# weikaolun/horovod-distributed-example

Hardware: AMD Instinct MI355X
Metric: images/sec (whole node) + scaling efficiency, ResNet-50 bf16 at 1/2/4/8 MI355X (higher is better)
Workload: dtype bf16; 1 GPU; model=ResNet-50, global_batch=2048, per_gpu_batch=2048, image=224, parallelism=dp1, optimizer=mivod FusedSGD via DistributedOptimizer, compression=none, transport=local, hip_graph=False

## Files before the change

### csrc/kernels/mv_gemm256.hip

```cpp
#include "mv_mfma.h"
#include "mv_gemm.h"

#include <cstdio>
#include <cstdlib>
#include <string>

namespace mv {
namespace g256 {

constexpr int BM = 256, BN = 256, BK = 64, NT = 512;
constexpr int HALF = 128 * BK;
constexpr int BUF = 4 * HALF;

#ifndef MV_G256_DIAG
#define MV_G256_DIAG 0
#endif
template <int N>
__device__ __forceinline__ void wait_vm() {
  if constexpr (!(MV_G256_DIAG & 1) || N == 0)
    mv::wait_vm<N>();
}
__device__ __forceinline__ void barrier() {
  if constexpr (MV_G256_DIAG & 8) return;
  __builtin_amdgcn_sched_barrier(0);
  raw_barrier();
  __builtin_amdgcn_sched_barrier(0);
}

struct Args {
  const __bf16* A;
  const __bf16* A2;
  const __bf16* B;
  __bf16* C;
  int64_t M;
  int N, K, K1, ntn;
  int64_t ntiles;
  int ds, H, W, Ho, Wo;
  int Cin, ks;
  int ph, pw, Kb;
  const float* shift;
  float* partial;
  const float* badd;
  const __bf16* xb;
  const float* mean;
  const float* sc;
  const float* bi;
  uint32_t abytes, a2bytes, bbytes;
  const __bf16* bias16;
};

struct Pixel {
  uint32_t n, ho, wo;
};
__device__ __forceinline__ Pixel pixel_of(uint32_t r, int Ho, int Wo) {
  const uint32_t hw = (uint32_t)(Ho * Wo);
  const uint32_t n = r / hw, rem = r - n * hw;
  const uint32_t ho = rem / (uint32_t)Wo;
  return Pixel{n, ho, rem - ho * (uint32_t)Wo};
}

template <int EPI>
constexpr int nvec() { return EPI == 1 ? 1 : EPI == 4 ? 4 : (EPI == 6 || EPI == 7) ? 1 : 0; }
constexpr int kVecFloats = 8192;

template <int EPI, int AMODE, int MT>
__global__ __launch_bounds__(NT, 1) void gemm256_kernel(Args p) {
  constexpr bool DM = AMODE == 3 || AMODE == 4;
  constexpr int BMv = MT * 32;
  constexpr int MH1 = MT - 4;
  constexpr int NV = nvec<EPI>();
  constexpr bool STATS = EPI == 1 || EPI == 4 || EPI == 7;
  constexpr bool BADD = EPI == 4 || EPI == 6;
  constexpr bool XB = EPI == 4 || EPI == 7;
  __shared__ __attribute__((aligned(16))) __bf16 smem[2 * BUF + (NV ? 2 * kVecFloats : 0)];
  float* vecs = reinterpret_cast<float*>(smem + 2 * BUF);
  float* stacc = vecs + 4 * BN;
  const int N = p.N;
  const int tid = threadIdx.x, lane = tid & 63;
  const int w = __builtin_amdgcn_readfirstlane(tid >> 6);
  const int wm = w >> 2, wn = w & 3;
  const int G = gridDim.x;
  int64_t tile = xcd_remap(blockIdx.x, G);
  if (tile >= p.ntiles) return;
  const int64_t tile0 = tile;
  const int nw0 = (int)(tile0 % p.ntn) * BN;

  uint32_t offa[2][2], offb[2][2];
  uint32_t offa2[2][2];
  uint32_t abase[2][2];
  uint32_t avalid[2];
  const uint32_t scb = (uint32_t)(((lane & 7) ^ ((lane >> 3) & 7)) * 16);
  const int KT = p.K / BK, KT1 = AMODE == 2 ? p.K1 / BK : KT;
  const int csteps = (AMODE == 3 || AMODE == 4) ? p.Cin / BK : 1;
  const bool cpow2 = (csteps & (csteps - 1)) == 0;
  const int cshift = __builtin_ctz((unsigned)csteps);
  auto set_src = [&](int64_t tl) {
    const int64_t mt = tl / p.ntn;
    const int nt = (int)(tl - mt * p.ntn);
#pragma unroll
    for (int i = 0; i < 2; ++i) {
      const int r = (2 * w + i) * 8 + (lane >> 3);
      const int sc = (lane & 7) ^ (r & 7);
#pragma unroll
      for (int h = 0; h < 2; ++h) {
        const int rr = (r & 63);
        int64_t row = mt * BMv + (r >> 6) * (MT * 16) + h * 64 +
                      ((h == 1 && rr >= 16 * MH1) ? rr - 16 * MH1 : rr);
        row = row < p.M ? row : p.M - 1;
        if constexpr (AMODE == 1) {
          const Pixel px = pixel_of((uint32_t)row, p.Ho, p.Wo);
          const int64_t n = px.n;
          const int ho = (int)px.ho, wo = (int)px.wo;
          row = (n * p.H + (int64_t)ho * p.ds) * p.W + (int64_t)wo * p.ds;
        }
        if constexpr (AMODE == 3) {
          const Pixel px = pixel_of((uint32_t)row, p.Ho, p.Wo);
          const int64_t n = px.n;
          const int ho = (int)px.ho, wo = (int)px.wo;
          const int pad = p.ks >> 1;
          const int hi0 = ho * p.ds - pad, wi0 = wo * p.ds - pad;
          uint32_t v = 0;
#pragma unroll
          for (int tr = 0; tr < 3; ++tr)
#pragma unroll
            for (int ts = 0; ts < 3; ++ts) {
              const bool ok = tr < p.ks && ts < p.ks && (unsigned)(hi0 + tr) < (unsigned)p.H &&
                              (unsigned)(wi0 + ts) < (unsigned)p.W;
              v |= (ok ? 1u : 0u) << (tr * p.ks + ts);
            }
          if (i == 0) avalid[h] = v;
          else avalid[h] |= v << 16;
          abase[h][i] =
              (uint32_t)(((((int64_t)n * p.H + hi0) * p.W + wi0) * p.Cin + sc * 8) * 2);
        }
        if constexpr (AMODE == 4) {
          const uint32_t hw = (uint32_t)(p.Ho * p.Wo);
          const int rem = (int)((uint32_t)row % hw);
          const int ci = (int)((uint32_t)rem / (uint32_t)p.Wo), cj = rem - ci * p.Wo;
          const bool r1 = ci + 1 < p.Ho, c1 = cj + 1 < p.Wo;
          const uint32_t v = 1u | (c1 ? 2u : 0u) | (r1 ? 4u : 0u) | (r1 && c1 ? 8u : 0u);
          if (i == 0) avalid[h] = v;
          else avalid[h] |= v << 16;
          abase[h][i] = (uint32_t)((row * p.Cin + sc * 8) * 2);
        }
        if constexpr (AMODE == 2) {
          offa[h][i] = (uint32_t)(row * (p.K1 * 2)) + scb;
          int64_t row2 = row;
          if (p.ds > 1) {
            const Pixel px = pixel_of((uint32_t)row, p.Ho, p.Wo);
            const int64_t n = px.n;
            const int ho = (int)px.ho, wo = (int)px.wo;
            row2 = (n * p.H + (int64_t)ho * p.ds) * p.W + (int64_t)wo * p.ds;
          }
          offa2[h][i] = (uint32_t)(row2 * ((p.K - p.K1) * 2)) + scb;
        } else {
          offa[h][i] = (uint32_t)((row * p.K + sc * 8) * 2);
        }
        const int col = nt * BN + (r >> 5) * 64 + h * 32 + (r & 31);
        offb[h][i] = (uint32_t)(((int64_t)col * (AMODE == 4 ? p.Kb : p.K) + sc * 8) * 2);
      }
    }
  };
  const __amdgpu_buffer_rsrc_t rsA = buffer_rsrc(p.A, p.abytes);
  const __amdgpu_buffer_rsrc_t rsA2 =
      buffer_rsrc(AMODE == 2 ? p.A2 : p.A, AMODE == 2 ? p.a2bytes : 0u);
  const __amdgpu_buffer_rsrc_t rsB = buffer_rsrc(p.B, p.bbytes);
  struct KInfo {
    uint32_t toff, boff;
    int tap;
  };
  auto kinfo = [&](int kt) -> KInfo {
    uint32_t toff = 0, boff = kt * (BK * 2);
    int tap = 0;
    if constexpr (AMODE == 3) {
      tap = cpow2 ? kt >> cshift : kt / csteps;
      const int c0 = (kt - tap * csteps) * BK;
      const int tr = p.ks == 3 ? (tap * 11) >> 5 : tap / p.ks;
      const int ts = tap - tr * p.ks;
      toff = (uint32_t)(((tr * p.W + ts) * p.Cin + c0) * 2);
    }
    if constexpr (AMODE == 4) {
      const int t = cpow2 ? kt >> cshift : kt / csteps;
      const int c0 = (kt - t * csteps) * BK;
      const int tR = p.pw ? t >> 1 : t, tS = p.pw ? t & 1 : 0;
      const int rr = p.ph ? 2 * tR : 1, ss = p.pw ? 2 * tS : 1;
      tap = 2 * tR + tS;
      toff = (uint32_t)(((tR * p.Wo + tS) * p.Cin + c0) * 2);
      boff = (uint32_t)(((rr * 3 + ss) * p.Cin + c0) * 2);
    }
    return KInfo{toff, boff, tap};
  };
  auto issue_k = [&](int slot, int buf, int kt, const KInfo& ki, int ione) {
    if ((MV_G256_DIAG & 2) && kt != 0) return;
    const uint32_t toff = ki.toff, boff = ki.boff;
    const int tap = ki.tap;
    const bool second = AMODE == 2 && kt >= KT1;
    auto one = [&](int i) {
      __bf16* dst = smem + buf * BUF + slot * HALF + (2 * w + i) * 512;
      uint32_t vo;
      if (slot >= 2) {
        vo = offb[slot - 2][i] + boff;
      } else if constexpr (AMODE == 3 || AMODE == 4) {
        vo = ((avalid[slot] >> (tap + 16 * i)) & 1u) ? abase[slot][i] + toff : 0xFFFFFFF0u;
      } else if constexpr (AMODE == 2) {
        vo = second ? offa2[slot][i] + (uint32_t)(kt - KT1) * (BK * 2)
                    : offa[slot][i] + (uint32_t)kt * (BK * 2);
      } else {
        vo = offa[slot][i] + (uint32_t)kt * (BK * 2);
      }
      blds16(slot >= 2 ? rsB : (second ? rsA2 : rsA), vo, dst);
    };
    if (ione >= 0) {
      one(ione);
    } else {
      one(0);
      one(1);
    }
  };
  auto issue = [&](int slot, int buf, int kt) { issue_k(slot, buf, kt, kinfo(kt), -1); };

  f32x4v acc[4][8];
#pragma unroll
  for (int a = 0; a < 4; ++a)
#pragma unroll
    for (int b = 0; b < 8; ++b) acc[a][b] = f32x4v{0.f, 0.f, 0.f, 0.f};
  bf16x8 af[4][2], bfr[2][2][2];
  const int rl = lane & 15, g = lane >> 4;

  int kt = 0;
  auto read_a = [&](int buf, int h) {
    if ((MV_G256_DIAG & 4) && kt != 0) return;
    const __bf16* base = smem + buf * BUF + h * HALF;
#pragma unroll
    for (int b = 0; b < 4; ++b)
      if (h == 0 || b < MH1)
#pragma unroll
        for (int kk = 0; kk < 2; ++kk)
          af[b][kk] =
              *reinterpret_cast<const bf16x8*>(base + swz64(wm * 64 + b * 16 + rl, kk * 4 + g));
  };
  auto read_b = [&](int buf, int h) {
    if ((MV_G256_DIAG & 4) && kt != 0) return;
    const __bf16* base = smem + buf * BUF + (2 + h) * HALF;
#pragma unroll
    for (int a = 0; a < 2; ++a)
#pragma unroll
      for (int kk = 0; kk < 2; ++kk)
        bfr[h][a][kk] =
            *reinterpret_cast<const bf16x8*>(base + swz64(wn * 32 + a * 16 + rl, kk * 4 + g));
  };
  auto mma = [&](int qm, int qn) {
    __builtin_amdgcn_s_setprio(1);
#pragma unroll
    for (int kk = 0; kk < 2; ++kk)
#pragma unroll
      for (int a = 0; a < 2; ++a)
#pragma unroll
        for (int b = 0; b < 4; ++b)
          if (qm == 0 || b < MH1)
            acc[qn * 2 + a][qm * 4 + b] = mfma(bfr[qn][a][kk], af[b][kk], acc[qn * 2 + a][qm * 4 + b]);
    __builtin_amdgcn_s_setprio(0);
  };
  auto mma_dm = [&](int qm0, int qn0, int qm1, int qn1, int npc, int step, auto&& piece) {
    __builtin_amdgcn_s_setprio(1);
    int t = 0;
#pragma unroll
    for (int h = 0; h < 2; ++h) {
      const int qm = h ? qm1 : qm0, qn = h ? qn1 : qn0;
#pragma unroll
      for (int kk = 0; kk < 2; ++kk)
#pragma unroll
        for (int a = 0; a < 2; ++a)
#pragma unroll
          for (int b = 0; b < 4; ++b)
            if (qm == 0 || b < MH1) {
              acc[qn * 2 + a][qm * 4 + b] =
                  mfma(bfr[qn][a][kk], af[b][kk], acc[qn * 2 + a][qm * 4 + b]);
              if (t >= 1 && (t - 1) % step == 0 && (t - 1) / step < npc) {
                __builtin_amdgcn_sched_barrier(0);
                piece((t - 1) / step);
                __builtin_amdgcn_sched_barrier(0);
              }
              ++t;
            }
    }
    __builtin_amdgcn_s_setprio(0);
  };
  auto out_row = [&](int64_t row) -> int64_t {
    if constexpr (AMODE != 4) {
      return row;
    } else {
      const Pixel px = pixel_of((uint32_t)row, p.Ho, p.Wo);
      return ((int64_t)px.n * p.H + 2 * px.ho + p.ph) * p.W + 2 * px.wo + p.pw;
    }
  };
  auto epilogue = [&](int64_t tl) {
    const int64_t mt = tl / p.ntn;
    const int n0 = (int)(tl - mt * p.ntn) * BN;
    const int64_t m0 = mt * BMv;
    float s1[2][8], s2[2][8];
#pragma unroll
    for (int q = 0; q < 2; ++q)
#pragma unroll
      for (int j = 0; j < 8; ++j) {
        s1[q][j] = 0.f;
        s2[q][j] = 0.f;
      }
    constexpr int XBB = EPI == 7 ? 4 : 2;
    uint4 xr[XBB][2];
#pragma unroll
    for (int b = 0; b < MT; ++b) {
      if (XB && (b % XBB) == 0) {
#pragma unroll
        for (int bb = 0; bb < XBB; ++bb) {
          const int64_t row = m0 + wm * (MT * 16) + (b + bb) * 16 + rl;
          const int64_t orow = out_row(row);
#pragma unroll
          for (int q = 0; q < 2; ++q) {
            const int c0 = n0 + wn * 64 + q * 32 + (g & 1) * 16 + (g >> 1) * 8;
            xr[bb][q] = (b + bb < MT && row < p.M) ? *reinterpret_cast<const uint4*>(p.xb + orow * N + c0)
                                  : uint4{0u, 0u, 0u, 0u};
          }
        }
      }
      const int64_t row = m0 + wm * (MT * 16) + b * 16 + rl;
      const bool in = row < p.M;
      const int64_t orow = out_row(row);
#pragma unroll
      for (int q = 0; q < 2; ++q) {
        f32x4v u = acc[2 * q][b], v = acc[2 * q + 1][b];
        if constexpr (BADD) {
          const int cu = n0 + wn * 64 + 2 * q * 16 + 4 * g;
          const f32x4v bu = *reinterpret_cast<const f32x4v*>(vecs + (cu - n0));
          const f32x4v bv = *reinterpret_cast<const f32x4v*>(vecs + (cu - n0) + 16);
          u += bu;
          v += bv;
        }
        uint32_t x0 = cvt_pk_bf16(u[0], u[1]), x1 = cvt_pk_bf16(u[2], u[3]);
        uint32_t y0 = cvt_pk_bf16(v[0], v[1]), y1 = cvt_pk_bf16(v[2], v[3]);
        const auto r0 = __builtin_amdgcn_permlane16_swap(x0, y0, false, false);
        const auto r1 = __builtin_amdgcn_permlane16_swap(x1, y1, false, false);
        uint32_t o[4] = {r0[0], r1[0], r0[1], r1[1]};
        const int c0 = n0 + wn * 64 + q * 32 + (g & 1) * 16 + (g >> 1) * 8;
        if constexpr (EPI == 1) {
          if (in) {
#pragma unroll
            for (int j = 0; j < 8; ++j) {
              const float f = (j & 1) ? __uint_as_float(o[j >> 1] & 0xffff0000u)
                                      : __uint_as_float(o[j >> 1] << 16);
              const float d = f - vecs[c0 - n0 + j];
              s1[q][j] += d;
              s2[q][j] += d * d;
            }
          }
        }
        if constexpr (EPI == 4) {
          if (in) {
            const uint32_t xw[4] = {xr[b % XBB][q].x, xr[b % XBB][q].y, xr[b % XBB][q].z, xr[b % XBB][q].w};
            const float* mean = vecs + BN - n0;
            const float* scv = vecs + 2 * BN - n0;
            const float* biv = vecs + 3 * BN - n0;
            float dv[8];
#pragma unroll
            for (int j = 0; j < 8; ++j) {
              const float f = (j & 1) ? __uint_as_float(o[j >> 1] & 0xffff0000u)
                                      : __uint_as_float(o[j >> 1] << 16);
              const float xv = (j & 1) ? __uint_as_float(xw[j >> 1] & 0xffff0000u)
                                       : __uint_as_float(xw[j >> 1] << 16);
              const float d = __builtin_fmaf(xv, scv[c0 + j], biv[c0 + j]) > 0.f ? f : 0.f;
              dv[j] = d;
              s1[q][j] += d;
              s2[q][j] += d * (xv - mean[c0 + j]);
            }
#pragma unroll
            for (int j = 0; j < 4; ++j) o[j] = cvt_pk_bf16(dv[2 * j], dv[2 * j + 1]);
          }
        }
        if constexpr (EPI == 7) {
          if (in) {
            const uint32_t xw[4] = {xr[b % XBB][q].x, xr[b % XBB][q].y, xr[b % XBB][q].z, xr[b % XBB][q].w};
            float dv[8];
#pragma unroll
            for (int j = 0; j < 8; ++j) {
              const float f = (j & 1) ? __uint_as_float(o[j >> 1] & 0xffff0000u)
                                      : __uint_as_float(o[j >> 1] << 16);
              const float xv = (j & 1) ? __uint_as_float(xw[j >> 1] & 0xffff0000u)
                                       : __uint_as_float(xw[j >> 1] << 16);
              const float d = f * gelu_grad(xv + vecs[c0 - n0 + j]);
              dv[j] = d;
              s1[q][j] += d;
            }
#pragma unroll
            for (int j = 0; j < 4; ++j) o[j] = cvt_pk_bf16(dv[2 * j], dv[2 * j + 1]);
          }
        }
        if (in && (EPI != 1 || p.C) && !(MV_G256_DIAG & 16)) {
          u32x4* dst = reinterpret_cast<u32x4*>(p.C + orow * N + c0);
          const u32x4 val{o[0], o[1], o[2], o[3]};
          if constexpr ((MV_G256_DIAG & 192) == 64) {
            __builtin_nontemporal_store(val, dst);
          } else if constexpr ((MV_G256_DIAG & 192) == 128) {
            asm volatile("global_store_dwordx4 %0, %1, off sc1" ::"v"(dst), "v"(val) : "memory");
          } else if constexpr ((MV_G256_DIAG & 192) == 192) {
            asm volatile("global_store_dwordx4 %0, %1, off sc0 sc1" ::"v"(dst), "v"(val) : "memory");
          } else {
            *dst = val;
          }
        }
      }
    }
    if constexpr (STATS) {
#pragma unroll
      for (int q = 0; q < 2; ++q)
#pragma unroll
        for (int j = 0; j < 8; ++j)
#pragma unroll
          for (int o = 1; o < 16; o <<= 1) {
            s1[q][j] += __shfl_xor(s1[q][j], o, kWave);
            s2[q][j] += __shfl_xor(s2[q][j], o, kWave);
          }
      if (rl == 0) {
        float* ac = stacc + wm * 2 * BN;
#pragma unroll
        for (int q = 0; q < 2; ++q) {
          const int cl = wn * 64 + q * 32 + (g & 1) * 16 + (g >> 1) * 8;
#pragma unroll
          for (int j = 0; j < 8; ++j) {
            ac[cl + j] += s1[q][j];
            ac[BN + cl + j] += s2[q][j];
          }
        }
      }
    }
#pragma unroll
    for (int a = 0; a < 4; ++a)
#pragma unroll
      for (int b = 0; b < 8; ++b) acc[a][b] = f32x4v{0.f, 0.f, 0.f, 0.f};
  };

  if constexpr (NV > 0) {
    for (int c = tid; c < BN; c += NT) {
      const int gc = nw0 + c;
      if constexpr (EPI == 1) vecs[c] = p.shift ? p.shift[gc] : 0.f;
      if constexpr (BADD) vecs[c] = p.badd ? p.badd[gc] : 0.f;
      if constexpr (EPI == 7) vecs[c] = p.bias16 ? (float)p.bias16[gc] : (p.badd ? p.badd[gc] : 0.f);
      if constexpr (EPI == 4) {
        vecs[BN + c] = p.mean[gc];
        vecs[2 * BN + c] = p.sc[gc];
        vecs[3 * BN + c] = p.bi[gc];
      }
    }
    if constexpr (STATS)
      for (int c = tid; c < 4 * BN; c += NT) stacc[c] = 0.f;
  }
  set_src(tile);
  issue(0, 0, 0);
  issue(2, 0, 0);
  issue(3, 0, 0);
  issue(1, 0, 0);
  if constexpr (DM) wait_vm<2>();
  else wait_vm<4>();
  barrier();
  if (wm == 1) barrier();

  int buf = 0;
  bool after = false;
  int64_t ntile = tile + G;
  for (;;) {
    const bool last_k = kt + 1 == KT;
    const bool more = !last_k || ntile < p.ntiles;
    const int nkt = last_k ? 0 : kt + 1;
    const int nb = buf ^ 1;
    if (last_k && more) set_src(ntile);
    if constexpr (DM) {
      const KInfo ki = kinfo(nkt);
      read_a(buf, 0);
      read_b(buf, 0);
      read_b(buf, 1);
      if (!after) wait_vm<0>();
      barrier();
      mma_dm(0, 0, 0, 1, 6, 5, [&](int j) {
        issue_k(j < 2 ? 0 : (j < 4 ? 2 : 3), nb, nkt, ki, j & 1);
      });
      barrier();
      read_a(buf, 1);
      wait_vm<0>();
      barrier();
      mma_dm(1, 1, 1, 0, 2, 10, [&](int j) { issue_k(1, nb, nkt, ki, j); });
      barrier();
      if (last_k) wait_vm<0>();
    } else {
      read_a(buf, 0);
      read_b(buf, 0);
      if (!more) {
        wait_vm<2>();
      } else if (last_k) {
        issue(0, nb, nkt);
        issue(2, nb, nkt);
        wait_vm<4>();
      } else {
        issue(0, nb, nkt);
        if (!after) wait_vm<4>();
      }
      barrier();
      mma(0, 0);
      barrier();
      read_b(buf, 1);
      if (!more) {
        wait_vm<0>();
      } else if (last_k) {
        issue(3, nb, nkt);
        issue(1, nb, nkt);
        wait_vm<8>();
      } else {
        issue(2, nb, nkt);
        if (!after) wait_vm<4>();
      }
      barrier();
      mma(0, 1);
      barrier();
      read_a(buf, 1);
      if (more && !last_k) issue(3, nb, nkt);
      barrier();
      mma(1, 1);
      barrier();
      if (more) {
        if (last_k) {
          wait_vm<0>();
        } else {
          issue(1, nb, nkt);
          wait_vm<4>();
        }
      }
      barrier();
      mma(1, 0);
      barrier();
    }
    buf = nb;
    after = last_k;
    if (last_k) {
      if constexpr (!(MV_G256_DIAG & 32)) epilogue(tile);
      if (!more) break;
      tile = ntile;
      ntile += G;
      kt = 0;
    } else {
      ++kt;
    }
  }
  if (wm == 0) barrier();
  if constexpr (STATS) {
    __syncthreads();
    float* pr = p.partial + ((tile0 / p.ntn) * 2 + wm) * 2 * N + nw0;
    const float* ac = stacc + wm * 2 * BN;
    pr[wn * 64 + lane] = ac[wn * 64 + lane];
    pr[N + wn * 64 + lane] = ac[BN + wn * 64 + lane];
  }
}


struct WArgs {
  const __bf16* X;
  const __bf16* DY;
  const __bf16* DY2;
  float* partial;
  int64_t M;
  int C, K, k1, ntc, ntiles, ms;
  int64_t per;
  int Cx, H, W, Ho, Wo, ds;
  uint32_t xbytes;
};

__device__ __forceinline__ int wf(int r) { return tr_swz8(r) << 1; }

__device__ __forceinline__ bf16x8 trp(const __bf16* pa, const __bf16* pb) {
  const s16x4 a = lds_tr4_asm(pa);
  const s16x4 b = lds_tr4_asm(pb);
  return cat8_shuffle(a, b);
}

template <int TAPS>
__global__ __launch_bounds__(NT, 1) void wgrad256_kernel(WArgs p) {
  constexpr bool DM = TAPS == 9;
  __shared__ __attribute__((aligned(16))) __bf16 smem[2 * BUF];
  const int tid = threadIdx.x, lane = tid & 63;
  const int w = __builtin_amdgcn_readfirstlane(tid >> 6);
  const int wc = w >> 2, wk = w & 3;
  const int t = xcd_remap(blockIdx.x, gridDim.x);
  const int split = t / p.ntiles, tl = t - split * p.ntiles;
  const int c0 = (tl % p.ntc) * 256, k0 = (tl / p.ntc) * 256;
  constexpr bool GATHER = TAPS != 1;
  const int tap = TAPS == 9 ? c0 / p.Cx : (TAPS == 2 ? 4 : 0);
  const int xc0 = TAPS == 9 ? c0 - tap * p.Cx : c0;
  const int tr = tap / 3, ts = tap - 3 * (tap / 3);
  const int64_t mb = (int64_t)split * p.per * BK;
  int64_t me = mb + p.per * BK;
  me = me < p.M ? me : p.M;
  const int KT = me > mb ? (int)((me - mb + BK - 1) / BK) : 0;

  int choff[4][2];
  const bool dual = p.k1 < p.K && k0 >= p.k1;
  const __bf16* dyb = dual ? p.DY2 : p.DY;
  const int ldy = dual ? p.K - p.k1 : p.k1;
  const int kb = dual ? k0 - p.k1 : k0;
#pragma unroll
  for (int i = 0; i < 2; ++i) {
    const int r = (2 * w + i) * 4 + (lane >> 4);
    const int lc = (lane & 15) ^ wf(r);
#pragma unroll
    for (int h = 0; h < 2; ++h) {
      choff[h][i] = xc0 + 128 * (lc >> 3) + 64 * h + 8 * (lc & 7);
      choff[2 + h][i] = kb + 64 * (lc >> 2) + 32 * h + 8 * (lc & 3);
    }
  }
  uint32_t xoff[2] = {0u, 0u};
  bool xok[2] = {false, false};
  uint32_t pn[2] = {0u, 0u}, pho[2] = {0u, 0u}, pwo[2] = {0u, 0u};
  uint32_t st_n = 0, st_ho = 0, st_wo = 0;
  if constexpr (GATHER) {
    const uint32_t hw = (uint32_t)(p.Ho * p.Wo);
    st_n = (uint32_t)BK / hw;
    const uint32_t r = (uint32_t)BK - st_n * hw;
    st_ho = r / (uint32_t)p.Wo;
    st_wo = r - st_ho * (uint32_t)p.Wo;
#pragma unroll
    for (int i = 0; i < 2; ++i) {
      const uint32_t r32 = (uint32_t)(mb + (2 * w + i) * 4 + (lane >> 4));
      pn[i] = r32 / hw;
      const uint32_t rem = r32 - pn[i] * hw;
      pho[i] = rem / (uint32_t)p.Wo;
      pwo[i] = rem - pho[i] * (uint32_t)p.Wo;
    }
  }
  const uint32_t nrow = me > mb ? (uint32_t)(me - mb) : 0u;
  const __amdgpu_buffer_rsrc_t rsX = buffer_rsrc(
      GATHER ? p.X : p.X + mb * p.C, GATHER ? p.xbytes : nrow * (uint32_t)(p.C * 2));
  const __amdgpu_buffer_rsrc_t rsD = buffer_rsrc(dyb + mb * ldy, nrow * (uint32_t)(ldy * 2));
  auto issue = [&](int slot, int buf, int kt, int ione = -1) {
#pragma unroll
    for (int i = 0; i < 2; ++i) {
      if (ione >= 0 && i != ione) continue;
      const uint32_t lrow = (uint32_t)(kt * BK + (2 * w + i) * 4 + (lane >> 4));
      uint32_t vo;
      bool xsrc = slot < 2;
      if (GATHER && slot < 2) {
        if (slot == 0) {
          const int hi = (int)pho[i] * p.ds - 1 + tr, wi = (int)pwo[i] * p.ds - 1 + ts;
          xok[i] = lrow < nrow && (unsigned)hi < (unsigned)p.H && (unsigned)wi < (unsigned)p.W;
          xoff[i] = ((pn[i] * (uint32_t)p.H + (uint32_t)hi) * (uint32_t)p.W + (uint32_t)wi) *
                    (uint32_t)(p.Cx * 2);
          pwo[i] += st_wo;
          const bool c1 = pwo[i] >= (uint32_t)p.Wo;
          pwo[i] = c1 ? pwo[i] - (uint32_t)p.Wo : pwo[i];
          pho[i] += st_ho + (c1 ? 1u : 0u);
          const bool c2 = pho[i] >= (uint32_t)p.Ho;
          pho[i] = c2 ? pho[i] - (uint32_t)p.Ho : pho[i];
          pn[i] += st_n + (c2 ? 1u : 0u);
        }
        vo = xok[i] ? xoff[i] + (uint32_t)(choff[slot][i] * 2) : 0xFFFFFFF0u;
      } else if (TAPS == 2 && dual) {
        vo = xok[i] ? xoff[i] + (uint32_t)(choff[slot][i] * 2) : 0xFFFFFFF0u;
        xsrc = true;
      } else {
        vo = lrow * (uint32_t)((slot < 2 ? p.C : ldy) * 2) + (uint32_t)(choff[slot][i] * 2);
      }
      blds16(xsrc ? rsX : rsD, vo, smem + buf * BUF + slot * HALF + (2 * w + i) * 512);
    }
  };

  f32x4v acc[4][8];
#pragma unroll
  for (int a = 0; a < 4; ++a)
#pragma unroll
    for (int b = 0; b < 8; ++b) acc[a][b] = f32x4v{0.f, 0.f, 0.f, 0.f};
  bf16x8 af[4][2], bfr[2][2][2];
  const int rl = lane & 15, g = lane >> 4;
  auto toff = [&](int r, int e) { return r * 128 + (((e >> 3) ^ wf(r)) << 3) + (e & 7); };
  auto read_a = [&](int buf, int h) {
    const __bf16* base = smem + buf * BUF + h * HALF;
#pragma unroll
    for (int b = 0; b < 4; ++b)
#pragma unroll
      for (int kk = 0; kk < 2; ++kk) {
        const int r = 32 * kk + 8 * g + (rl >> 2), e = 64 * wc + 16 * b + 4 * (rl & 3);
        af[b][kk] = trp(base + toff(r, e), base + toff(r + 4, e));
      }
  };
  auto read_b = [&](int buf, int h) {
    const __bf16* base = smem + buf * BUF + (2 + h) * HALF;
#pragma unroll
    for (int a = 0; a < 2; ++a)
#pragma unroll
      for (int kk = 0; kk < 2; ++kk) {
        const int r = 32 * kk + 8 * g + (rl >> 2), e = 32 * wk + 16 * a + 4 * (rl & 3);
        bfr[h][a][kk] = trp(base + toff(r, e), base + toff(r + 4, e));
      }
  };
  auto mma = [&](int qc, int qk) {
    lds_wait();
    __builtin_amdgcn_s_setprio(1);
#pragma unroll
    for (int kk = 0; kk < 2; ++kk)
#pragma unroll
      for (int a = 0; a < 2; ++a)
#pragma unroll
        for (int b = 0; b < 4; ++b)
          acc[qk * 2 + a][qc * 4 + b] = mfma(af[b][kk], bfr[qk][a][kk], acc[qk * 2 + a][qc * 4 + b]);
    __builtin_amdgcn_s_setprio(0);
  };
  auto mma_dm = [&](int qc0, int qk0, int qc1, int qk1, int npc, int step, auto&& piece) {
    lds_wait();
    __builtin_amdgcn_s_setprio(1);
    int t = 0;
#pragma unroll
    for (int h = 0; h < 2; ++h) {
      const int qc = h ? qc1 : qc0, qk = h ? qk1 : qk0;
#pragma unroll
      for (int kk = 0; kk < 2; ++kk)
#pragma unroll
        for (int a = 0; a < 2; ++a)
#pragma unroll
          for (int b = 0; b < 4; ++b) {
            acc[qk * 2 + a][qc * 4 + b] = mfma(af[b][kk], bfr[qk][a][kk], acc[qk * 2 + a][qc * 4 + b]);
            if (t >= 1 && (t - 1) % step == 0 && (t - 1) / step < npc) {
              __builtin_amdgcn_sched_barrier(0);
              piece((t - 1) / step);
              __builtin_amdgcn_sched_barrier(0);
            }
            ++t;
          }
    }
    __builtin_amdgcn_s_setprio(0);
  };

  if (KT > 0 && DM) {
    issue(0, 0, 0);
    issue(2, 0, 0);
    issue(3, 0, 0);
    issue(1, 0, 0);
    wait_vm<2>();
    barrier();
    if (wc == 1) barrier();
    for (int kt = 0; kt < KT; ++kt) {
      const int buf = kt & 1, nb = buf ^ 1;
      read_a(buf, 0);
      read_b(buf, 0);
      read_b(buf, 1);
      wait_vm<0>();
      barrier();
      mma_dm(0, 0, 0, 1, 6, 5, [&](int j) { issue(j < 2 ? 0 : (j < 4 ? 2 : 3), nb, kt + 1, j & 1); });
      barrier();
      read_a(buf, 1);
      wait_vm<0>();
      barrier();
      mma_dm(1, 1, 1, 0, 2, 10, [&](int j) { issue(1, nb, kt + 1, j); });
      barrier();
    }
    wait_vm<0>();
    if (wc == 0) barrier();
  } else if (KT > 0) {
    issue(0, 0, 0);
    issue(2, 0, 0);
    issue(3, 0, 0);
    issue(1, 0, 0);
    wait_vm<2>();
    barrier();
    if (wc == 1) barrier();
    for (int kt = 0; kt < KT; ++kt) {
      const int buf = kt & 1, nb = buf ^ 1;
      const bool more = kt + 1 < KT;
      read_a(buf, 0);
      read_b(buf, 0);
      read_b(buf, 1);
      if (more) {
        issue(0, nb, kt + 1);
        issue(2, nb, kt + 1);
        issue(3, nb, kt + 1);
        wait_vm<6>();
      } else {
        wait_vm<0>();
      }
      barrier();
      mma(0, 0);
      mma(0, 1);
      barrier();
      read_a(buf, 1);
      if (more) {
        issue(1, nb, kt + 1);
        wait_vm<2>();
      }
      barrier();
      mma(1, 1);
      mma(1, 0);
      barrier();
    }
    if (wc == 0) barrier();
  }
  float* pp = p.partial + (int64_t)split * p.K * p.C;
#pragma unroll
  for (int a = 0; a < 4; ++a)
#pragma unroll
    for (int b = 0; b < 8; ++b) {
      const int k = k0 + 64 * wk + 16 * a + rl, c = c0 + 128 * wc + 16 * b + 4 * g;
      *reinterpret_cast<f32x4v*>(pp + (int64_t)k * p.C + c) = acc[a][b];
    }
}

}
}

static bool g256_trace() {
  static const bool v = [] {
    const char* e = std::getenv("MIVOD_G256");
    return e && std::string(e) == "trace";
  }();
  return v;
}

static int g256_bm(int64_t M, int N) { return N == 256 && M % 224 == 0 ? 224 : 256; }

bool mv_gemm256_supported(int64_t M, int N, int K) {
  return M > 0 && N % 256 == 0 && K % 64 == 0 && K >= 64 &&
         (M + 255) / 256 * (N / 256) < (int64_t(1) << 31) && M * K * 2 < (int64_t(1) << 32) &&
         (int64_t)N * K * 2 < (int64_t(1) << 32);
}

static int64_t g256_grid(int64_t M, int N) {
  const int64_t ntn = N / mv::g256::BN, bm = g256_bm(M, N);
  const int64_t ntiles = (M + bm - 1) / bm * ntn, cus = mv::num_cus();
  const int64_t g = (ntiles < cus ? ntiles : cus) / ntn * ntn;
  return g > ntn ? g : ntn;
}

int64_t mv_gemm256_partials(int64_t M, int N) {
  return 2 * (g256_grid(M, N) / (N / mv::g256::BN));
}

template <int EPI, int AMODE>
static void g256_launch(mv::g256::Args a, hipStream_t st) {
  using namespace mv::g256;
  const int bm = g256_bm(a.M, a.N);
  if (g256_trace())
    std::fprintf(stderr, "[g256] gemm256 EPI %d AMODE %d M %lld N %d K %d Cin %d ks %d ds %d H %d W %d C %d\n",
                 EPI, AMODE, (long long)a.M, a.N, a.K, a.Cin, a.ks, a.ds, a.H, a.W, a.C ? 1 : 0);
  a.ntn = a.N / BN;
  a.ntiles = (a.M + bm - 1) / bm * a.ntn;
  const dim3 grid((unsigned)g256_grid(a.M, a.N));
  if (bm == 224) hipLaunchKernelGGL((gemm256_kernel<EPI, AMODE, 7>), grid, dim3(NT), 0, st, a);
  else hipLaunchKernelGGL((gemm256_kernel<EPI, AMODE, 8>), grid, dim3(NT), 0, st, a);
}

template <int TAPS>
static void w256_launch(const mv::g256::WArgs& a, hipStream_t st) {
  using namespace mv::g256;
  const dim3 grid((unsigned)(a.ntiles * a.ms));
  if (g256_trace())
    std::fprintf(stderr, "[g256] wgrad256 TAPS %d M %lld C %d K %d k1 %d Cx %d H %d W %d ds %d grid %u\n",
                 TAPS, (long long)a.M, a.C, a.K, a.k1, a.Cx, a.H, a.W, a.ds, grid.x);
  hipLaunchKernelGGL((wgrad256_kernel<TAPS>), grid, dim3(NT), 0, st, a);
}

bool mv_gemm256_nt(const void* A, const void* B, void* C, int64_t M, int N, int K,
                   const float* shift, float* partial, hipStream_t st) {
  using namespace mv::g256;
  if (!mv_gemm256_supported(M, N, K) || (partial && N > kVecFloats) || (!C && !partial))
    return false;
  Args a{};
  a.A = (const __bf16*)A;
  a.B = (const __bf16*)B;
  a.C = (__bf16*)C;
  a.M = M;
  a.N = N;
  a.K = K;
  a.shift = shift;
  a.partial = partial;
  a.abytes = (uint32_t)(M * K * 2);
  a.bbytes = (uint32_t)((int64_t)N * K * 2);
  if (partial) g256_launch<1, 0>(a, st);
  else g256_launch<0, 0>(a, st);
  return true;
}

bool mv_gemm256_strided(const void* X, const void* B, void* C, int Nb, int H, int W, int K, int N,
                        int ds, const float* shift, float* partial, hipStream_t st) {
  using namespace mv::g256;
  const int Ho = (H - 1) / ds + 1, Wo = (W - 1) / ds + 1;
  const int64_t M = (int64_t)Nb * Ho * Wo;
  if (ds < 1 || !mv_gemm256_supported(M, N, K) || (partial && N > kVecFloats) ||
      (int64_t)Nb * H * W * K * 2 >= (int64_t(1) << 32))
    return false;
  Args a{};
  a.A = (const __bf16*)X;
  a.B = (const __bf16*)B;
  a.C = (__bf16*)C;
  a.M = M;
  a.N = N;
  a.K = K;
  a.ds = ds;
  a.H = H;
  a.W = W;
  a.Ho = Ho;
  a.Wo = Wo;
  a.shift = shift;
  a.partial = partial;
  a.abytes = (uint32_t)((int64_t)Nb * H * W * K * 2);
  a.bbytes = (uint32_t)((int64_t)N * K * 2);
  if (partial) g256_launch<1, 1>(a, st);
  else g256_launch<0, 1>(a, st);
  return true;
}

bool mv_gemm256_dual(const void* A1, const void* A2, const void* B, const float* badd, void* D,
                     int64_t M, int K1, int K2, int N, const void* xb, const float* mean,
                     const float* scale, const float* bias, float* partial, hipStream_t st,
                     int ds, int H, int W) {
  using namespace mv::g256;
  const int K = K1 + K2;
  if (K1 % 64 || K2 % 64 || !mv_gemm256_supported(M, N, K) || 4 * N > kVecFloats) return false;
  Args a{};
  if (ds > 1) {
    a.Ho = (H - 1) / ds + 1;
    a.Wo = (W - 1) / ds + 1;
    const int64_t hw = (int64_t)a.Ho * a.Wo;
    if (H < 1 || W < 1 || M % hw != 0 || (M / hw) * H * W * (int64_t)K2 * 2 >= (int64_t(1) << 32))
      return false;
    a.ds = ds;
    a.H = H;
    a.W = W;
  }
  a.A = (const __bf16*)A1;
  a.A2 = (const __bf16*)A2;
  a.B = (const __bf16*)B;
  a.C = (__bf16*)D;
  a.M = M;
  a.N = N;
  a.K = K;
  a.K1 = K1;
  a.badd = badd;
  a.xb = (const __bf16*)xb;
  a.mean = mean;
  a.sc = scale;
  a.bi = bias;
  a.partial = partial;
  a.abytes = (uint32_t)(M * K1 * 2);
  a.a2bytes = (uint32_t)((ds > 1 ? M / ((int64_t)a.Ho * a.Wo) * H * W : M) * K2 * 2);
  a.bbytes = (uint32_t)((int64_t)N * K * 2);
  if (partial) g256_launch<4, 2>(a, st);
  else g256_launch<6, 2>(a, st);
  return true;
}

bool mv_gemm256_gelu_bwd(const void* dY, const void* Wt, const void* pre, const void* bias16,
                         void* D, float* partial, int64_t M, int N, int K, hipStream_t st) {
  using namespace mv::g256;
  if (!mv_gemm256_supported(M, N, K) || N > kVecFloats || !dY || !Wt || !pre || !bias16 || !D ||
      !partial || M * (int64_t)K * 2 >= (int64_t(1) << 32))
    return false;
  Args a{};
  a.A = (const __bf16*)dY;
  a.B = (const __bf16*)Wt;
  a.C = (__bf16*)D;
  a.M = M;
  a.N = N;
  a.K = K;
  a.xb = (const __bf16*)pre;
  a.bias16 = (const __bf16*)bias16;
  a.partial = partial;
  a.abytes = (uint32_t)(M * K * 2);
  a.bbytes = (uint32_t)((int64_t)N * K * 2);
  g256_launch<7, 0>(a, st);
  return true;
}

bool mv_conv256_supported(int N, int H, int W, int Cin, int Cout, int ks, int stride) {
  const int Ho = (H - 1) / stride + 1, Wo = (W - 1) / stride + 1;
  const int64_t M = (int64_t)N * Ho * Wo;
  return (ks == 1 || ks == 3) && stride >= 1 && stride <= 2 && Cin % 64 == 0 && Cin > 0 &&
         (int64_t)N * H * W * Cin * 2 < (int64_t(1) << 32) - 16 &&
         Cout % 256 == 0 && Cout <= mv::g256::kVecFloats / 4 && M > 0 &&
         (M + 255) / 256 * (Cout / 256) < (int64_t(1) << 31) &&
         (int64_t)Cout * ks * ks * Cin * 2 < (int64_t(1) << 32);
}

bool mv_conv256(const void* X, const void* Wt, void* Y, int Nb, int H, int W, int Cin, int Cout,
                int ks, int stride, const float* shift, float* partial, const void* bn_x,
                const float* bn_vec, hipStream_t st) {
  using namespace mv::g256;
  if (!mv_conv256_supported(Nb, H, W, Cin, Cout, ks, stride) || (bn_x && !partial)) return false;
  Args a{};
  a.A = (const __bf16*)X;
  a.B = (const __bf16*)Wt;
  a.C = (__bf16*)Y;
  a.Ho = (H - 1) / stride + 1;
  a.Wo = (W - 1) / stride + 1;
  a.M = (int64_t)Nb * a.Ho * a.Wo;
  a.N = Cout;
  a.K = ks * ks * Cin;
  a.ds = stride;
  a.H = H;
  a.W = W;
  a.Cin = Cin;
  a.ks = ks;
// ... 176 lines not shown
```

Measured before the change: 19080 images/sec.

## Split-K the last partial wave of gemm256 tiles with a reduction tail kernel

When the persistent gemm256 grid leaves a small final wave of tiles (at most half the grid), those remaining tiles are split along K across S workgroups. Each writes fp32 partial accumulators to a cached workspace, and a new tail kernel sums the slabs and runs the shared epilogue, including the BN stats partial rows. The epilogue is factored into a reusable device function. The aim is to fix wave-quantization imbalance, at the cost of an extra launch, workspace traffic and a device allocation on first use (skipped during graph capture).

```diff
diff --git a/csrc/kernels/mv_gemm256.hip b/csrc/kernels/mv_gemm256.hip
--- a/csrc/kernels/mv_gemm256.hip
+++ b/csrc/kernels/mv_gemm256.hip
@@ -1,9 +1,12 @@
 #include "mv_mfma.h"
 #include "mv_gemm.h"
 
+#include <algorithm>
 #include <cstdio>
 #include <cstdlib>
+#include <mutex>
 #include <string>
+#include <vector>
 
 namespace mv {
 namespace g256 {
@@ -47,7 +50,11 @@
   const float* bi;
   uint32_t abytes, a2bytes, bbytes;
   const __bf16* bias16;
+  int64_t nfull;
+  int S, tailr;
+  float* ws;
 };
+constexpr int kSlab = 8 * 32 * 256;
 
 struct Pixel {
   uint32_t n, ho, wo;
@@ -63,7 +70,174 @@
 constexpr int nvec() { return EPI == 1 ? 1 : EPI == 4 ? 4 : (EPI == 6 || EPI == 7) ? 1 : 0; }
 constexpr int kVecFloats = 8192;
 
-template <int EPI, int AMODE, int MT>
+template <int AMODE>
+__device__ __forceinline__ int64_t out_row(const Args& p, int64_t row) {
+  if constexpr (AMODE != 4) {
+    return row;
+  } else {
+    const Pixel px = pixel_of((uint32_t)row, p.Ho, p.Wo);
+    return ((int64_t)px.n * p.H + 2 * px.ho + p.ph) * p.W + 2 * px.wo + p.pw;
+  }
+}
+
+template <int EPI, int AMODE, int MT, int NB, bool TAIL>
+__device__ __forceinline__ void tile_epilogue(const Args& p, f32x4v (&acc)[4][8], int64_t tl,
+                                              const float* vecs, float* ac, int acs, int wm,
+                                              int wn, int lane, int b0) {
+  constexpr int BMv = MT * 32;
+  constexpr bool STATS = EPI == 1 || EPI == 4 || EPI == 7;
+  constexpr bool BADD = EPI == 4 || EPI == 6;
+  constexpr bool XB = EPI == 4 || EPI == 7;
+  const int N = p.N;
+  const int rl = lane & 15, g = lane >> 4;
+  const int64_t mt = tl / p.ntn;
+  const int n0 = (int)(tl - mt * p.ntn) * BN;
+  const int64_t m0 = mt * BMv;
+  float s1[2][8], s2[2][8];
+#pragma unroll
+  for (int q = 0; q < 2; ++q)
+#pragma unroll
+    for (int j = 0; j < 8; ++j) {
+      s1[q][j] = 0.f;
+      s2[q][j] = 0.f;
+    }
+  constexpr int XBB = EPI == 7 ? 4 : 2;
+  uint4 xr[XBB][2];
+#pragma unroll
+  for (int b = 0; b < NB; ++b) {
+    if (XB && (b % XBB) == 0) {
+#pragma unroll
+      for (int bb = 0; bb < XBB; ++bb) {
+        const int64_t row = m0 + wm * (MT * 16) + (b0 + b + bb) * 16 + rl;
+        const int64_t orow = out_row<AMODE>(p, row);
+#pragma unroll
+        for (int q = 0; q < 2; ++q) {
+          const int c0 = n0 + wn * 64 + q * 32 + (g & 1) * 16 + (g >> 1) * 8;
+          xr[bb][q] = (b + bb < NB && row < p.M) ? *reinterpret_cast<const uint4*>(p.xb + orow * N + c0)
+                                : uint4{0u, 0u, 0u, 0u};
+        }
+      }
+    }
+    const int64_t row = m0 + wm * (MT * 16) + (b0 + b) * 16 + rl;
+    const bool in = row < p.M;
+    const int64_t orow = out_row<AMODE>(p, row);
+#pragma unroll
+    for (int q = 0; q < 2; ++q) {
+      f32x4v u = acc[2 * q][b], v = acc[2 * q + 1][b];
+      if constexpr (BADD) {
+        const int cu = n0 + wn * 64 + 2 * q * 16 + 4 * g;
+        const f32x4v bu = *reinterpret_cast<const f32x4v*>(vecs + (cu - n0));
+        const f32x4v bv = *reinterpret_cast<const f32x4v*>(vecs + (cu - n0) + 16);
+        u += bu;
+        v += bv;
+      }
+      uint32_t x0 = cvt_pk_bf16(u[0], u[1]), x1 = cvt_pk_bf16(u[2], u[3]);
+      uint32_t y0 = cvt_pk_bf16(v[0], v[1]), y1 = cvt_pk_bf16(v[2], v[3]);
+      const auto r0 = __builtin_amdgcn_permlane16_swap(x0, y0, false, false);
+      const auto r1 = __builtin_amdgcn_permlane16_swap(x1, y1, false, false);
+      uint32_t o[4] = {r0[0], r1[0], r0[1], r1[1]};
+      const int c0 = n0 + wn * 64 + q * 32 + (g & 1) * 16 + (g >> 1) * 8;
+      if constexpr (EPI == 1) {
+        if (in) {
+#pragma unroll
+          for (int j = 0; j < 8; ++j) {
+            const float f = (j & 1) ? __uint_as_float(o[j >> 1] & 0xffff0000u)
+                                    : __uint_as_float(o[j >> 1] << 16);
+            const float d = f - vecs[c0 - n0 + j];
+            s1[q][j] += d;
+            s2[q][j] += d * d;
+          }
+        }
+      }
+      if constexpr (EPI == 4) {
+        if (in) {
+          const uint32_t xw[4] = {xr[b % XBB][q].x, xr[b % XBB][q].y, xr[b % XBB][q].z, xr[b % XBB][q].w};
+          const float* mean = vecs + BN - n0;
+          const float* scv = vecs + 2 * BN - n0;
+          const float* biv = vecs + 3 * BN - n0;
+          float dv[8];
+#pragma unroll
+          for (int j = 0; j < 8; ++j) {
+            const float f = (j & 1) ? __uint_as_float(o[j >> 1] & 0xffff0000u)
+                                    : __uint_as_float(o[j >> 1] << 16);
+            const float xv = (j & 1) ? __uint_as_float(xw[j >> 1] & 0xffff0000u)
+                                     : __uint_as_float(xw[j >> 1] << 16);
+            const float d = __builtin_fmaf(xv, scv[c0 + j], biv[c0 + j]) > 0.f ? f : 0.f;
+            dv[j] = d;
+            s1[q][j] += d;
+            s2[q][j] += d * (xv - mean[c0 + j]);
+          }
+#pragma unroll
+          for (int j = 0; j < 4; ++j) o[j] = cvt_pk_bf16(dv[2 * j], dv[2 * j + 1]);
+        }
+      }
+      if constexpr (EPI == 7) {
+        if (in) {
+          const uint32_t xw[4] = {xr[b % XBB][q].x, xr[b % XBB][q].y, xr[b % XBB][q].z, xr[b % XBB][q].w};
+          float dv[8];
+#pragma unroll
+          for (int j = 0; j < 8; ++j) {
+            const float f = (j & 1) ? __uint_as_float(o[j >> 1] & 0xffff0000u)
+                                    : __uint_as_float(o[j >> 1] << 16);
+            const float xv = (j & 1) ? __uint_as_float(xw[j >> 1] & 0xffff0000u)
+                                     : __uint_as_float(xw[j >> 1] << 16);
+            const float d = f * gelu_grad(xv + vecs[c0 - n0 + j]);
+            dv[j] = d;
+            s1[q][j] += d;
+          }
+#pragma unroll
+          for (int j = 0; j < 4; ++j) o[j] = cvt_pk_bf16(dv[2 * j], dv[2 * j + 1]);
+        }
+      }
+      if (in && (EPI != 1 || p.C) && !(MV_G256_DIAG & 16)) {
+        u32x4* dst = reinterpret_cast<u32x4*>(p.C + orow * N + c0);
+        const u32x4 val{o[0], o[1], o[2], o[3]};
+        if constexpr ((MV_G256_DIAG & 192) == 64) {
+          __builtin_nontemporal_store(val, dst);
+        } else if constexpr ((MV_G256_DIAG & 192) == 128) {
+          asm volatile("global_store_dwordx4 %0, %1, off sc1" ::"v"(dst), "v"(val) : "memory");
+        } else if constexpr ((MV_G256_DIAG & 192) == 192) {
+          asm volatile("global_store_dwordx4 %0, %1, off sc0 sc1" ::"v"(dst), "v"(val) : "memory");
+        } else {
+          *dst = val;
+        }
+      }
+    }
+  }
+  if constexpr (STATS) {
+#pragma unroll
+    for (int q = 0; q < 2; ++q)
+#pragma unroll
+      for (int j = 0; j < 8; ++j)
+#pragma unroll
+        for (int o = 1; o < 16; o <<= 1) {
+          s1[q][j] += __shfl_xor(s1[q][j], o, kWave);
+          s2[q][j] += __shfl_xor(s2[q][j], o, kWave);
+        }
+    if (rl == 0) {
+#pragma unroll
+      for (int q = 0; q < 2; ++q) {
+        const int cl = wn * 64 + q * 32 + (g & 1) * 16 + (g >> 1) * 8;
+#pragma unroll
+        for (int j = 0; j < 8; ++j) {
+          if constexpr (TAIL) {
+            ac[cl + j] = s1[q][j];
+            ac[acs + cl + j] = s2[q][j];
+          } else {
+            ac[cl + j] += s1[q][j];
+            ac[acs + cl + j] += s2[q][j];
+          }
+        }
+      }
+    }
+  }
+#pragma unroll
+  for (int a = 0; a < 4; ++a)
+#pragma unroll
+    for (int b = 0; b < 8; ++b) acc[a][b] = f32x4v{0.f, 0.f, 0.f, 0.f};
+}
+
+template <int EPI, int AMODE, int MT, bool SPLIT>
 __global__ __launch_bounds__(NT, 1) void gemm256_kernel(Args p) {
   constexpr bool DM = AMODE == 3 || AMODE == 4;
   constexpr int BMv = MT * 32;
@@ -286,158 +460,32 @@
     }
     __builtin_amdgcn_s_setprio(0);
   };
-  auto out_row = [&](int64_t row) -> int64_t {
-    if constexpr (AMODE != 4) {
-      return row;
-    } else {
-      const Pixel px = pixel_of((uint32_t)row, p.Ho, p.Wo);
-      return ((int64_t)px.n * p.H + 2 * px.ho + p.ph) * p.W + 2 * px.wo + p.pw;
-    }
-  };
   auto epilogue = [&](int64_t tl) {
-    const int64_t mt = tl / p.ntn;
-    const int n0 = (int)(tl - mt * p.ntn) * BN;
-    const int64_t m0 = mt * BMv;
-    float s1[2][8], s2[2][8];
-#pragma unroll
-    for (int q = 0; q < 2; ++q)
-#pragma unroll
-      for (int j = 0; j < 8; ++j) {
-        s1[q][j] = 0.f;
-        s2[q][j] = 0.f;
-      }
-    constexpr int XBB = EPI == 7 ? 4 : 2;
-    uint4 xr[XBB][2];
-#pragma unroll
-    for (int b = 0; b < MT; ++b) {
-      if (XB && (b % XBB) == 0) {
-#pragma unroll
-        for (int bb = 0; bb < XBB; ++bb) {
-          const int64_t row = m0 + wm * (MT * 16) + (b + bb) * 16 + rl;
-          const int64_t orow = out_row(row);
-#pragma unroll
-          for (int q = 0; q < 2; ++q) {
-            const int c0 = n0 + wn * 64 + q * 32 + (g & 1) * 16 + (g >> 1) * 8;
-            xr[bb][q] = (b + bb < MT && row < p.M) ? *reinterpret_cast<const uint4*>(p.xb + orow * N + c0)
-                                  : uint4{0u, 0u, 0u, 0u};
-          }
-        }
-      }
-      const int64_t row = m0 + wm * (MT * 16) + b * 16 + rl;
-      const bool in = row < p.M;
-      const int64_t orow = out_row(row);
-#pragma unroll
-      for (int q = 0; q < 2; ++q) {
-        f32x4v u = acc[2 * q][b], v = acc[2 * q + 1][b];
-        if constexpr (BADD) {
-          const int cu = n0 + wn * 64 + 2 * q * 16 + 4 * g;
-          const f32x4v bu = *reinterpret_cast<const f32x4v*>(vecs + (cu - n0));
-          const f32x4v bv = *reinterpret_cast<const f32x4v*>(vecs + (cu - n0) + 16);
-          u += bu;
-          v += bv;
-        }
-        uint32_t x0 = cvt_pk_bf16(u[0], u[1]), x1 = cvt_pk_bf16(u[2], u[3]);
-        uint32_t y0 = cvt_pk_bf16(v[0], v[1]), y1 = cvt_pk_bf16(v[2], v[3]);
-        const auto r0 = __builtin_amdgcn_permlane16_swap(x0, y0, false, false);
-        const auto r1 = __builtin_amdgcn_permlane16_swap(x1, y1, false, false);
-        uint32_t o[4] = {r0[0], r1[0], r0[1], r1[1]};
-        const int c0 = n0 + wn * 64 + q * 32 + (g & 1) * 16 + (g >> 1) * 8;
-        if constexpr (EPI == 1) {
-          if (in) {
-#pragma unroll
-            for (int j = 0; j < 8; ++j) {
-              const float f = (j & 1) ? __uint_as_float(o[j >> 1] & 0xffff0000u)
-                                      : __uint_as_float(o[j >> 1] << 16);
-              const float d = f - vecs[c0 - n0 + j];
-              s1[q][j] += d;
-              s2[q][j] += d * d;
-            }
-          }
-        }
-        if constexpr (EPI == 4) {
-          if (in) {
-            const uint32_t xw[4] = {xr[b % XBB][q].x, xr[b % XBB][q].y, xr[b % XBB][q].z, xr[b % XBB][q].w};
-            const float* mean = vecs + BN - n0;
-            const float* scv = vecs + 2 * BN - n0;
-            const float* biv = vecs + 3 * BN - n0;
-            float dv[8];
-#pragma unroll
-            for (int j = 0; j < 8; ++j) {
-              const float f = (j & 1) ? __uint_as_float(o[j >> 1] & 0xffff0000u)
-                                      : __uint_as_float(o[j >> 1] << 16);
-              const float xv = (j & 1) ? __uint_as_float(xw[j >> 1] & 0xffff0000u)
-                                       : __uint_as_float(xw[j >> 1] << 16);
-              const float d = __builtin_fmaf(xv, scv[c0 + j], biv[c0 + j]) > 0.f ? f : 0.f;
-              dv[j] = d;
-              s1[q][j] += d;
-              s2[q][j] += d * (xv - mean[c0 + j]);
-            }
-#pragma unroll
-            for (int j = 0; j < 4; ++j) o[j] = cvt_pk_bf16(dv[2 * j], dv[2 * j + 1]);
-          }
-        }
-        if constexpr (EPI == 7) {
-          if (in) {
-            const uint32_t xw[4] = {xr[b % XBB][q].x, xr[b % XBB][q].y, xr[b % XBB][q].z, xr[b % XBB][q].w};
-            float dv[8];
-#pragma unroll
-            for (int j = 0; j < 8; ++j) {
-              const float f = (j & 1) ? __uint_as_float(o[j >> 1] & 0xffff0000u)
-                                      : __uint_as_float(o[j >> 1] << 16);
-              const float xv = (j & 1) ? __uint_as_float(xw[j >> 1] & 0xffff0000u)
-                                       : __uint_as_float(xw[j >> 1] << 16);
-              const float d = f * gelu_grad(xv + vecs[c0 - n0 + j]);
-              dv[j] = d;
-              s1[q][j] += d;
-            }
-#pragma unroll
-            for (int j = 0; j < 4; ++j) o[j] = cvt_pk_bf16(dv[2 * j], dv[2 * j + 1]);
-          }
-        }
-        if (in && (EPI != 1 || p.C) && !(MV_G256_DIAG & 16)) {
-          u32x4* dst = reinterpret_cast<u32x4*>(p.C + orow * N + c0);
-          const u32x4 val{o[0], o[1], o[2], o[3]};
-          if constexpr ((MV_G256_DIAG & 192) == 64) {
-            __builtin_nontemporal_store(val, dst);
-          } else if constexpr ((MV_G256_DIAG & 192) == 128) {
-            asm volatile("global_store_dwordx4 %0, %1, off sc1" ::"v"(dst), "v"(val) : "memory");
-          } else if constexpr ((MV_G256_DIAG & 192) == 192) {
-            asm volatile("global_store_dwordx4 %0, %1, off sc0 sc1" ::"v"(dst), "v"(val) : "memory");
-          } else {
-            *dst = val;
-          }
-        }
-      }
-    }
-    if constexpr (STATS) {
-#pragma unroll
-      for (int q = 0; q < 2; ++q)
-#pragma unroll
-        for (int j = 0; j < 8; ++j)
-#pragma unroll
-          for (int o = 1; o < 16; o <<= 1) {
-            s1[q][j] += __shfl_xor(s1[q][j], o, kWave);
-            s2[q][j] += __shfl_xor(s2[q][j], o, kWave);
-          }
-      if (rl == 0) {
-        float* ac = stacc + wm * 2 * BN;
-#pragma unroll
-        for (int q = 0; q < 2; ++q) {
-          const int cl = wn * 64 + q * 32 + (g & 1) * 16 + (g >> 1) * 8;
-#pragma unroll
-          for (int j = 0; j < 8; ++j) {
-            ac[cl + j] += s1[q][j];
-            ac[BN + cl + j] += s2[q][j];
-          }
-        }
-      }
-    }
+    tile_epilogue<EPI, AMODE, MT, MT, false>(p, acc, tl, vecs, stacc + wm * 2 * BN, BN, wm, wn,
+                                             lane, 0);
+  };
+  int64_t ptile = -1;
+  int pk0 = 0, pk1 = 0, pslab = 0;
+  if (SPLIT && p.S > 1) {
+    const int q = (int)(tile0 / p.ntn), r = q / p.S, s = q - r * p.S;
+    if (r < p.tailr) {
+      const int j = r * p.ntn + (int)(tile0 % p.ntn);
+      ptile = p.nfull + j;
+      pk0 = s * KT / p.S;
+      pk1 = (s + 1) * KT / p.S;
+      pslab = j * p.S + s;
+    }
+  }
+  auto spill = [&]() {
+    char* slab = reinterpret_cast<char*>(p.ws + (int64_t)pslab * kSlab + w * (32 * 256));
+    uint32_t voff = (uint32_t)lane * 16u;
+    asm volatile("" : "+v"(voff));
 #pragma unroll
     for (int a = 0; a < 4; ++a)
 #pragma unroll
-      for (int b = 0; b < 8; ++b) acc[a][b] = f32x4v{0.f, 0.f, 0.f, 0.f};
-  };
-
+      for (int b = 0; b < MT; ++b)
+        *reinterpret_cast<f32x4v*>(slab + (a * 8 + b) * 1024 + voff) = acc[a][b];
+  };
   if constexpr (NV > 0) {
     for (int c = tid; c < BN; c += NT) {
       const int gc = nw0 + c;
@@ -466,12 +514,16 @@
   int buf = 0;
   bool after = false;
   int64_t ntile = tile + G;
+  int kend = KT;
+  bool part = false;
   for (;;) {
-    const bool last_k = kt + 1 == KT;
-    const bool more = !last_k || ntile < p.ntiles;
-    const int nkt = last_k ? 0 : kt + 1;
+    const bool last_k = kt + 1 == kend;
+    const bool nwhole = ntile < (SPLIT ? p.nfull : p.ntiles);
+    const bool npart = SPLIT && !nwhole && !part && ptile >= 0;
+    const bool more = !last_k || nwhole || npart;
+    const int nkt = last_k ? (npart ? pk0 : 0) : kt + 1;
     const int nb = buf ^ 1;
-    if (last_k && more) set_src(ntile);
+    if (last_k && more) set_src(npart ? ptile : ntile);
     if constexpr (DM) {
       const KInfo ki = kinfo(nkt);
       read_a(buf, 0);
@@ -539,15 +591,24 @@
     buf = nb;
     after = last_k;
     if (last_k) {
-      if constexpr (!(MV_G256_DIAG & 32)) epilogue(tile);
+      if constexpr (!(MV_G256_DIAG & 32))
+        if (!SPLIT || !part) epilogue(tile);
       if (!more) break;
-      tile = ntile;
-      ntile += G;
-      kt = 0;
+      if (SPLIT && npart) {
+        tile = ptile;
+        part = true;
+        kt = pk0;
+        kend = pk1;
+      } else {
+        tile = ntile;
+        ntile += G;
+        kt = 0;
+      }
     } else {
       ++kt;
     }
   }
+  if (SPLIT && part) spill();
   if (wm == 0) barrier();
   if constexpr (STATS) {
     __syncthreads();
@@ -555,6 +616,73 @@
     const float* ac = stacc + wm * 2 * BN;
     pr[wn * 64 + lane] = ac[wn * 64 + lane];
     pr[N + wn * 64 + lane] = ac[BN + wn * 64 + lane];
+    if (!SPLIT && p.tailr > 0 && tile0 < p.ntn) {
+      float* z = p.partial + (int64_t)(G / p.ntn) * 4 * N + nw0;
+      for (int i = tid; i < p.tailr * 4 * BN; i += NT) z[(int64_t)(i / BN) * N + (i % BN)] = 0.f;
+    }
+  }
+}
+
+template <int EPI, int AMODE, int MT>
+__global__ __launch_bounds__(NT) void gemm256_tail_kernel(Args p, int prow0) {
+  constexpr int NV = nvec<EPI>();
+  constexpr bool STATS = EPI == 1 || EPI == 4 || EPI == 7;
+  constexpr bool BADD = EPI == 4 || EPI == 6;
+  __shared__ __attribute__((aligned(16))) float lds[4 * BN + (STATS ? 8 * 2 * BN : 0)];
+  float* vecs = lds;
+  float* st = lds + 4 * BN;
+  const int tid = threadIdx.x, lane = tid & 63;
+  const int b = __builtin_amdgcn_readfirstlane(tid >> 6);
+  const int j = blockIdx.x >> 3, w = blockIdx.x & 7;
+  const int wm = w >> 2, wn = w & 3;
+  const int64_t tl = p.nfull + j;
+  const int r = j / p.ntn, n0 = (j - r * p.ntn) * BN;
+  if constexpr (NV > 0) {
+    for (int c = tid; c < BN; c += NT) {
+      const int gc = n0 + c;
+      if constexpr (EPI == 1) vecs[c] = p.shift ? p.shift[gc] : 0.f;
+      if constexpr (BADD) vecs[c] = p.badd ? p.badd[gc] : 0.f;
+      if constexpr (EPI == 7) vecs[c] = p.bias16 ? (float)p.bias16[gc] : (p.badd ? p.badd[gc] : 0.f);
+      if constexpr (EPI == 4) {
+        vecs[BN + c] = p.mean[gc];
+        vecs[2 * BN + c] = p.sc[gc];
+        vecs[3 * BN + c] = p.bi[gc];
+      }
+    }
+    __syncthreads();
+  }
+  if (b < MT) {
+    f32x4v acc[4][8];
+#pragma unroll
+    for (int a = 0; a < 4; ++a)
+#pragma unroll
+      for (int i = 0; i < 8; ++i) acc[a][i] = f32x4v{0.f, 0.f, 0.f, 0.f};
+    const float* slab = p.ws + (int64_t)j * p.S * kSlab + w * (32 * 256) + b * 256 + lane * 4;
+    for (int s0 = 0; s0 < p.S; s0 += 8) {
+      f32x4v t[8][4];
+#pragma unroll
+      for (int i = 0; i < 8; ++i)
+#pragma unroll
+        for (int a = 0; a < 4; ++a)
+          t[i][a] = s0 + i < p.S
+                        ? *reinterpret_cast<const f32x4v*>(slab + (int64_t)(s0 + i) * kSlab + a * 8 * 256)
+                        : f32x4v{0.f, 0.f, 0.f, 0.f};
+#pragma unroll
+      for (int i = 0; i < 8; ++i)
+#pragma unroll
+        for (int a = 0; a < 4; ++a) acc[a][0] += t[i][a];
+    }
+    tile_epilogue<EPI, AMODE, MT, 1, true>(p, acc, tl, vecs, st + b * 2 * BN, BN, wm, wn, lane, b);
+  }
+  if constexpr (STATS) {
+    __syncthreads();
+    if (tid < 128) {
+      const int col = wn * 64 + (tid & 63), h = tid >> 6;
+      float v = 0.f;
+#pragma unroll
+      for (int i = 0; i < MT; ++i) v += st[i * 2 * BN + h * BN + col];
+      p.partial[((int64_t)(prow0 + 2 * r + wm) * 2 + h) * p.N + n0 + col] = v;
+    }
   }
 }
 
@@ -832,22 +960,98 @@
   return g > ntn ? g : ntn;
 }
 
+#ifndef MV_G256_TAIL_SMAX
+#define MV_G256_TAIL_SMAX 8
+#endif
+constexpr int kTailSMax = MV_G256_TAIL_SMAX, kTailKMin = 2;
+struct G256Tail {
+  int64_t G, full, L;
+  bool active;
+};
+static G256Tail g256_tail(int64_t M, int N) {
+  const int64_t ntn = N / mv::g256::BN, bm = g256_bm(M, N);
+  const int64_t ntiles = (M + bm - 1) / bm * ntn, G = g256_grid(M, N);
+  const int64_t full = ntiles / G, L = ntiles - full * G;
+  return G256Tail{G, full, L, full >= 1 && L > 0 && 2 * L <= G};
+}
+
+constexpr int kTailMaxFull = 6, kTailMinKT = 24;
+static bool g256_tail_pays(int64_t full, int S, int KT) {
+  (void)S;
+  return full <= kTailMaxFull && (full < 3 || KT >= kTailMinKT);
+}
+
 int64_t mv_gemm256_partials(int64_t M, int N) {
-  return 2 * (g256_grid(M, N) / (N / mv::g256::BN));
+  const G256Tail t = g256_tail(M, N);
+  const int64_t ntn = N / mv::g256::BN;
+  return 2 * (t.G / ntn) + (t.active ? 2 * (t.L / ntn) : 0);
+}
+
+static float* g256_workspace(hipStream_t st, int64_t G) {
+  struct Ent {
+    int dev;
+    hipStream_t st;
+    int64_t G;
+    float* p;
+  };
+  static std::mutex mu;
+  static std::vector<Ent> ents;
+  int dev = 0;
+  if (hipGetDevice(&dev) != hipSuccess) return nullptr;
+  std::lock_guard<std::mutex> lk(mu);
+  for (const Ent& e : ents)
+    if (e.dev == dev && e.st == st && e.G >= G) return e.p;
+  hipStreamCaptureStatus cs = hipStreamCaptureStatusNone;
+  if (hipStreamIsCapturing(st, &cs) != hipSuccess || cs != hipStreamCaptureStatusNone) {
+    (void)hipGetLastError();
+    return nullptr;
+  }
+  void* p = nullptr;
+  if (hipMalloc(&p, (size_t)G * mv::g256::kSlab * sizeof(float)) != hipSuccess) {
+    (void)hipGetLastError();
+    return nullptr;
+  }
+  ents.push_back(Ent{dev, st, G, (float*)p});
+  return (float*)p;
 }
 
 template <int EPI, int AMODE>
 static void g256_launch(mv::g256::Args a, hipStream_t st) {
   using namespace mv::g256;
   const int bm = g256_bm(a.M, a.N);
-  if (g256_trace())
-    std::fprintf(stderr, "[g256] gemm256 EPI %d AMODE %d M %lld N %d K %d Cin %d ks %d ds %d H %d W %d C %d\n",
-                 EPI, AMODE, (long long)a.M, a.N, a.K, a.Cin, a.ks, a.ds, a.H, a.W, a.C ? 1 : 0);
   a.ntn = a.N / BN;
   a.ntiles = (a.M + bm - 1) / bm * a.ntn;
-  const dim3 grid((unsigned)g256_grid(a.M, a.N));
-  if (bm == 224) hipLaunchKernelGGL((gemm256_kernel<EPI, AMODE, 7>), grid, dim3(NT), 0, st, a);
-  else hipLaunchKernelGGL((gemm256_kernel<EPI, AMODE, 8>), grid, dim3(NT), 0, st, a);
+  const G256Tail t = g256_tail(a.M, a.N);
+  int S = 1;
+  if (t.active) {
+    S = (int)std::min<int64_t>(std::min<int64_t>(t.G / t.L, kTailSMax), a.K / BK / kTailKMin);
+    if (S > 1 && !g256_tail_pays(t.full, S, a.K / BK)) S = 1;
+    if (S > 1 && !(a.ws = g256_workspace(st, t.G))) S = 1;
+  }
+  const bool split = S > 1;
+  a.S = split ? S : 1;
+  a.nfull = split ? t.full * t.G : a.ntiles;
+  a.tailr = t.active ? (int)(t.L / a.ntn) : 0;
+  if (g256_trace())
+    std::fprintf(stderr, "[g256] gemm256 EPI %d AMODE %d M %lld N %d K %d Cin %d ks %d ds %d H %d W %d C %d S %d\n",
+                 EPI, AMODE, (long long)a.M, a.N, a.K, a.Cin, a.ks, a.ds, a.H, a.W, a.C ? 1 : 0,
+                 a.S);
+  const dim3 grid((unsigned)t.G);
+  if (bm == 224) {
+    if (split) hipLaunchKernelGGL((gemm256_kernel<EPI, AMODE, 7, true>), grid, dim3(NT), 0, st, a);
+    else hipLaunchKernelGGL((gemm256_kernel<EPI, AMODE, 7, false>), grid, dim3(NT), 0, st, a);
+  } else {
+    if (split) hipLaunchKernelGGL((gemm256_kernel<EPI, AMODE, 8, true>), grid, dim3(NT), 0, st, a);
+    else hipLaunchKernelGGL((gemm256_kernel<EPI, AMODE, 8, false>), grid, dim3(NT), 0, st, a);
+  }
+  const int prow0 = (int)(2 * (t.G / a.ntn));
+  if (split) {
+    const dim3 tgrid((unsigned)(t.L * 8));
+    if (bm == 224)
+      hipLaunchKernelGGL((gemm256_tail_kernel<EPI, AMODE, 7>), tgrid, dim3(NT), 0, st, a, prow0);
+    else
+      hipLaunchKernelGGL((gemm256_tail_kernel<EPI, AMODE, 8>), tgrid, dim3(NT), 0, st, a, prow0);
+  }
 }
 
 template <int TAPS>
```

Result: no change. 19180 images/sec (median of 6 runs) (+0.5%).
